# ChenFengTsai/dreamerv3-torch

Hardware: AMD Instinct MI355X
Metric: imagination-steps/sec (higher is better)
Workload: dtype f32; 1 GPU; cfg2: dmc_vision 64x64x3 synthetic replay, RSSM deter=512 hidden=512 stoch=32x32, continuous actor (6), imag_gradient dynamics, batch 16 x seq 64 per GPU, horizon 15; one step = full Dreamer._train update (world model + actor + critic fwd/bwd, gradient all-reduce, 3x clip+Adam); global_batch=16, seq_len=64, horizon=15, parallelism=dp1

## Files before the change

### dreamerv3-torch_amd/csrc/conv.hip

```cpp
#include <stdlib.h>

#include "mfma_gemm.h"
#include "l16_tile.h"
#include "dv3_common.h"

namespace dv3 {

struct FastDiv {
  int d, shift;
  __host__ __device__ static FastDiv make(int d) {
    FastDiv f{d, -1};
    if (d > 0 && (d & (d - 1)) == 0) {
      int s = 0;
      while ((1 << s) < d) ++s;
      f.shift = s;
    }
    return f;
  }
  __device__ __forceinline__ long quot(long x) const { return shift >= 0 ? (x >> shift) : x / d; }
  __device__ __forceinline__ int rem(long x) const { return shift >= 0 ? (int)(x & (d - 1)) : (int)(x % d); }
  __device__ __forceinline__ int quot(int x) const { return shift >= 0 ? (x >> shift) : x / d; }
  __device__ __forceinline__ int rem(int x) const { return shift >= 0 ? (x & (d - 1)) : x % d; }
};

// ... 509 lines not shown
  f32x4n acc[2][RN];
#pragma unroll
  for (int t = 0; t < 2; ++t)
#pragma unroll
    for (int c = 0; c < RN; ++c) acc[t][c] = (f32x4n){0.f, 0.f, 0.f, 0.f};
  const int chunks = (K + 15) >> 4;
  f32x4n a0[2], b0[RN], a1[2], b1[RN];
  float m0[2], m1[2];
  auto load = [&](f32x4n (&a)[2], f32x4n (&b)[RN], float (&msk)[2], int c) {
    if (c >= chunks) return;
    const int k = (c << 4) + 4 * q;
    const int tap = dC.quot(k), ci = dC.rem(k);
    const int ky = tap >> 2, kx = tap & 3;
#pragma unroll
    for (int t = 0; t < 2; ++t) {
      const int iy = y0[t] + ky, ix = x0[t] + kx;
      const bool ok = base[t] >= 0 && iy >= 0 && iy < p.H && ix >= 0 && ix < p.W;
      const float* src = ok ? p.x + base[t] + ((long)iy * p.W + ix) * p.Ci + ci : p.x;
      a[t] = *reinterpret_cast<const f32x4u*>(src);
      msk[t] = ok ? 1.f : 0.f;
    }
#pragma unroll
    for (int cc = 0; cc < RN; ++cc) b[cc] = *reinterpret_cast<const f32x4u*>(wrow[cc] + k);
  };
  auto compute = [&](const f32x4n (&a)[2], const f32x4n (&b)[RN], const float (&msk)[2], int c) {
    if (c >= chunks) return;
#pragma unroll
    for (int g = 0; g < 4; ++g)
#pragma unroll
      for (int t = 0; t < 2; ++t) {
        const float av = a[t][g] * msk[t];
#pragma unroll
        for (int cc = 0; cc < RN; ++cc)
          acc[t][cc] = __builtin_amdgcn_mfma_f32_16x16x4f32(av, b[cc][g] * bmask[cc], acc[t][cc], 0, 0, 0);
      }
  };
  load(a0, b0, m0, 0);
  for (int c = 0; c < chunks; c += 2) {
    load(a1, b1, m1, c + 1);
    compute(a0, b0, m0, c);
    load(a0, b0, m0, c + 2);
    compute(a1, b1, m1, c + 1);
  }
#pragma unroll
  for (int t = 0; t < 2; ++t)
#pragma unroll
    for (int r = 0; r < 4; ++r) {
      const long m = row0 + 16 * t + 4 * q + r;
      if (m >= M) continue;
      float* orow = p.y + m * p.Co;
#pragma unroll
      for (int cc = 0; cc < RN; ++cc) {
        const int co = 16 * cc + i;
        if (co < p.Co) orow[co] = p.accumulate ? (orow[co] + acc[t][cc][r]) : acc[t][cc][r];
      }
    }
}

struct WgradParams {
  const float* dy;
  const float* x;
  float* dw;
  int Nimg, H, W, Ci, Co;
  int tiles_m, tiles_n, splits, chunk;
  int xcd_group;
};

template <class TS, bool C3 = false>
__global__ __launch_bounds__(kThreads) void conv_wgrad_kernel(WgradParams p) {
  __shared__ __attribute__((aligned(16))) float lds[TS::lds_floats];
  using ATile = DenseTile<TS::BM, TS::BK, false>;
  using BTile = WgradBTile<TS::BN, TS::BK, C3>;
  const int OH = p.H / 2, OW = p.W / 2;
  const long rows = (long)p.Nimg * OH * OW;
  DenseOperand<false> aop{p.dy, nullptr, (long)p.Co, 0, p.Co, (int)rows, (int)rows, true};
  WgradB bop{p.x, p.H, p.W, p.Ci, OH, OW, rows, 16 * p.Ci, FastDiv::make(OW), FastDiv::make(OH),
             FastDiv::make(p.Ci), FastDiv::make(4 * p.Ci)};
  const int tiles = p.tiles_m * p.tiles_n;
  int tile, split;
  if (p.xcd_group) {
    const int xcd = blockIdx.x & 7, j = blockIdx.x >> 3;
    split = (j / tiles) * 8 + xcd;
    tile = j % tiles;
    if (split >= p.splits) return;
  } else {
    tile = blockIdx.x % tiles;
    split = blockIdx.x / tiles;
  }
  const int m0 = (tile / p.tiles_n) * TS::BM, n0 = (tile % p.tiles_n) * TS::BN;
  const long kb = (long)split * p.chunk;
  long ke = kb + p.chunk;
  if (ke > rows) ke = rows;
  f32x16 acc[TS::TM][TS::TN];
  bool owner;
  mfma_mainloop<TS, ATile, BTile>(aop, bop, m0, n0, (int)kb, (int)ke, lds, acc, owner);
  if (kb >= ke || !owner) return;
  const int tid = threadIdx.x, wave = (tid >> 6) % (TS::WM * TS::WN), lane = tid & 63;
  const int wm = wave / TS::WN, wn = wave % TS::WN, col_l = lane & 31, h = lane >> 5;
#pragma unroll
  for (int a = 0; a < TS::TM; ++a)
#pragma unroll
    for (int b = 0; b < TS::TN; ++b) {
      const int j = n0 + (wn * TS::TN + b) * 32 + col_l;
      if (j >= 16 * p.Ci) continue;
#pragma unroll
      for (int r = 0; r < 16; ++r) {
        const int co = m0 + (wm * TS::TM + a) * 32 + (r & 3) + 8 * (r >> 2) + 4 * h;
        if (co < p.Co) atomicAdd(p.dw + (long)co * (16 * p.Ci) + j, acc[a][b][r]);
      }
    }
}

__global__ void unpack_conv_wgrad_kernel(float* __restrict__ packed, float* __restrict__ dw, int Co, int Ci) {
  const long total = (long)Co * Ci * 16;
  for (long i = (long)blockIdx.x * blockDim.x + threadIdx.x; i < total; i += (long)gridDim.x * blockDim.x) {
    const int ci = (int)(i % Ci);
    long t = i / Ci;
    const int kx = (int)(t % 4);
    t /= 4;
    const int ky = (int)(t % 4);
    const long co = t / 4;
    dw[((co * Ci + ci) * 4 + ky) * 4 + kx] += packed[i];
    packed[i] = 0.f;
  }
}

__global__ void pack_conv_w_kernel(const float* __restrict__ w, float* __restrict__ wp, int Co, int Ci) {
  const long total = (long)Co * Ci * 16;
  for (long i = (long)blockIdx.x * blockDim.x + threadIdx.x; i < total; i += (long)gridDim.x * blockDim.x) {
    const int ci = (int)(i % Ci);
    long t = i / Ci;
    const int kx = (int)(t % 4);
    t /= 4;
    const int ky = (int)(t % 4);
    const long co = t / 4;
    wp[i] = w[((co * Ci + ci) * 4 + ky) * 4 + kx];
  }
}
__global__ void pack_convT_w_kernel(const float* __restrict__ w, float* __restrict__ wp, int Ci, int Co) {
  const long total = 4L * Co * 4 * Ci;
  for (long i = (long)blockIdx.x * blockDim.x + threadIdx.x; i < total; i += (long)gridDim.x * blockDim.x) {
    const int ci = (int)(i % Ci);
    long t = i / Ci;
    const int b = (int)(t % 2);
    t /= 2;
    const int a = (int)(t % 2);
    t /= 2;
    const int co = (int)(t % Co);
    const int cls = (int)(t / Co);
    const int py = cls >> 1, px = cls & 1;
    const int ky = 1 - py + 2 * a, kx = 1 - px + 2 * b;
    wp[i] = w[(((long)ci * Co + co) * 4 + ky) * 4 + kx];
  }
}


typedef float f4a __attribute__((ext_vector_type(4), aligned(4)));

template <int CW>
__global__ __launch_bounds__(256) void conv_s2_c3_kernel(const float* __restrict__ x, const float* __restrict__ w,
                                                         float* __restrict__ y, int Nimg, int H, int W,
                                                         int accumulate) {
  const int OH = H / 2, OW = W / 2;
  const long total = (long)Nimg * OH * OW;
  for (long p = (long)blockIdx.x * blockDim.x + threadIdx.x; p < total; p += (long)gridDim.x * blockDim.x) {
    const int ox = (int)(p % OW);
    const long t = p / OW;
    const int oy = (int)(t % OH);
    const long n = t / OH;
    float in[4][12];
#pragma unroll
    for (int ky = 0; ky < 4; ++ky) {
      const int iy = 2 * oy - 1 + ky;
      const bool rowok = iy >= 0 && iy < H;
      const float* row = x + ((n * H + (rowok ? iy : 0)) * W) * 3;
#pragma unroll
      for (int kx = 0; kx < 4; ++kx) {
        const int ix = 2 * ox - 1 + kx;
        const bool ok = rowok && ix >= 0 && ix < W;
        const float* q = row + (ok ? ix : 0) * 3;
        const float m = ok ? 1.f : 0.f;
        in[ky][kx * 3 + 0] = q[0] * m;
        in[ky][kx * 3 + 1] = q[1] * m;
        in[ky][kx * 3 + 2] = q[2] * m;
      }
    }
    float* out = y + p * CW;
#pragma unroll 1
    for (int c0 = 0; c0 < CW; c0 += 4) {
      f4a acc = {0.f, 0.f, 0.f, 0.f};
#pragma unroll
      for (int e = 0; e < 4; ++e) {
        const float* wc = w + (long)(c0 + e) * 48;
        float a = 0.f;
#pragma unroll
        for (int c = 0; c < 3; ++c)
#pragma unroll
          for (int ky = 0; ky < 4; ++ky)
#pragma unroll
            for (int kx = 0; kx < 4; ++kx) a += in[ky][kx * 3 + c] * wc[(c * 4 + ky) * 4 + kx];
        acc[e] = a;
      }
      f4a* o = reinterpret_cast<f4a*>(out + c0);
      if (accumulate) acc += *o;
      *o = acc;
    }
  }
}

template <int CW>
__global__ __launch_bounds__(256) void conv_s2_c3_mfma_kernel(const float* __restrict__ x, const float* __restrict__ w,
                                                              float* __restrict__ y, int Nimg, int H, int W,
                                                              int accumulate) {
  constexpr int LD = 52, TN = CW / 16;
  __shared__ __attribute__((aligned(16))) float As[128 * LD];
  __shared__ __attribute__((aligned(16))) float Bs[CW * LD];
  const int tid = threadIdx.x, wave = tid >> 6, lane = tid & 63;
  const int i = lane & 15, q = lane >> 4;
  const int OH = H / 2, OW = W / 2;
  const long total = (long)Nimg * OH * OW;
  const long p0 = (long)blockIdx.x * 128;
  for (int e = tid; e < CW * 48; e += 256) {
    const int co = e / 48, r = e - co * 48;
    const int c = r >> 4, ky = (r >> 2) & 3, kx = r & 3;
    Bs[co * LD + ky * 12 + kx * 3 + c] = w[e];
  }
  {
    const int pl = tid >> 1, kyb = (tid & 1) * 2;
    const long p = p0 + pl;
    const bool pv = p < total;
    const long pc = pv ? p : 0;
    const int ox = (int)(pc % OW);
    const long t = pc / OW;
    const int oy = (int)(t % OH);
    const long n = t / OH;
    const bool edge = (ox == 0) || (ox == OW - 1);
#pragma unroll
    for (int kk = 0; kk < 2; ++kk) {
      const int ky = kyb + kk;
      const int iy = 2 * oy - 1 + ky;
      const bool rowok = pv && iy >= 0 && iy < H;
      float* dst = &As[pl * LD + ky * 12];
      f32x4 v0 = {0.f, 0.f, 0.f, 0.f}, v1 = v0, v2 = v0;
      if (rowok) {
        const float* row = x + ((n * H + iy) * W) * 3;
        if (!edge) {
          const float* src = row + (2 * ox - 1) * 3;
          v0 = *reinterpret_cast<const f32x4u*>(src);
          v1 = *reinterpret_cast<const f32x4u*>(src + 4);
          v2 = *reinterpret_cast<const f32x4u*>(src + 8);
        } else {
          float tmp[12];
#pragma unroll
          for (int j = 0; j < 12; ++j) {
            const int ix = 2 * ox - 1 + j / 3;
            tmp[j] = (ix >= 0 && ix < W) ? row[ix * 3 + j % 3] : 0.f;
          }
          v0 = (f32x4){tmp[0], tmp[1], tmp[2], tmp[3]};
          v1 = (f32x4){tmp[4], tmp[5], tmp[6], tmp[7]};
          v2 = (f32x4){tmp[8], tmp[9], tmp[10], tmp[11]};
        }
      }
      *reinterpret_cast<f32x4*>(dst) = v0;
      *reinterpret_cast<f32x4*>(dst + 4) = v1;
      *reinterpret_cast<f32x4*>(dst + 8) = v2;
    }
  }
  __syncthreads();
  f32x4 acc[2][TN];
#pragma unroll
  for (int a = 0; a < 2; ++a)
#pragma unroll
    for (int b = 0; b < TN; ++b) acc[a][b] = (f32x4){0.f, 0.f, 0.f, 0.f};
#pragma unroll
  for (int c = 0; c < 3; ++c) {
    f32x4 af[2], bf[TN];
#pragma unroll
    for (int a = 0; a < 2; ++a) af[a] = *reinterpret_cast<const f32x4*>(&As[(wave * 32 + 16 * a + i) * LD + 16 * c + 4 * q]);
#pragma unroll
    for (int b = 0; b < TN; ++b) bf[b] = *reinterpret_cast<const f32x4*>(&Bs[(16 * b + i) * LD + 16 * c + 4 * q]);
#pragma unroll
    for (int g = 0; g < 4; ++g)
#pragma unroll
      for (int a = 0; a < 2; ++a)
#pragma unroll
        for (int b = 0; b < TN; ++b)
          acc[a][b] = __builtin_amdgcn_mfma_f32_16x16x4f32(af[a][g], bf[b][g], acc[a][b], 0, 0, 0);
  }
#pragma unroll
  for (int a = 0; a < 2; ++a)
#pragma unroll
    for (int b = 0; b < TN; ++b)
#pragma unroll
      for (int r = 0; r < 4; ++r) {
        const long p = p0 + wave * 32 + 16 * a + 4 * q + r;
        if (p < total) {
          float* o = y + p * CW + 16 * b + i;
          const float v = acc[a][b][r];
          *o = accumulate ? (*o + v) : v;
        }
      }
}

template <int CW>
__global__ __launch_bounds__(256) void convT_s2_c3_kernel(const float* __restrict__ x, const float* __restrict__ w,
                                                          const float* __restrict__ bias, float out_add,
                                                          float* __restrict__ y, int Nimg, int IH, int IW,
                                                          int accumulate) {
  const long total = (long)Nimg * IH * IW;
  const int OW = 2 * IW, OH = 2 * IH;
  for (long p = (long)blockIdx.x * blockDim.x + threadIdx.x; p < total; p += (long)gridDim.x * blockDim.x) {
    const int x2 = (int)(p % IW);
    const long t = p / IW;
    const int y2 = (int)(t % IH);
    const long n = t / IH;
    float acc[2][2][3];
#pragma unroll
    for (int py = 0; py < 2; ++py)
#pragma unroll
      for (int px = 0; px < 2; ++px)
#pragma unroll
        for (int co = 0; co < 3; ++co) acc[py][px][co] = 0.f;
#pragma unroll 1
    for (int c0 = 0; c0 < CW; c0 += 4) {
      f4a in[3][3];
#pragma unroll
      for (int dy = 0; dy < 3; ++dy)
#pragma unroll
        for (int dx = 0; dx < 3; ++dx) {
          const int iy = y2 + dy - 1, ix = x2 + dx - 1;
          const bool ok = iy >= 0 && iy < IH && ix >= 0 && ix < IW;
          const float* q = x + (((n * IH + (ok ? iy : 0)) * IW + (ok ? ix : 0)) * CW) + c0;
          in[dy][dx] = *reinterpret_cast<const f4a*>(q) * (ok ? 1.f : 0.f);
        }
#pragma unroll
      for (int e = 0; e < 4; ++e) {
        const float* wc = w + (long)(c0 + e) * 48;
#pragma unroll
        for (int py = 0; py < 2; ++py)
#pragma unroll
          for (int a = 0; a < 2; ++a)
#pragma unroll
            for (int px = 0; px < 2; ++px)
#pragma unroll
              for (int b = 0; b < 2; ++b) {
                const float v = in[py - a + 1][px - b + 1][e];
                const int ky = 1 - py + 2 * a, kx = 1 - px + 2 * b;
#pragma unroll
                for (int co = 0; co < 3; ++co) acc[py][px][co] += v * wc[(co * 4 + ky) * 4 + kx];
              }
      }
    }
    const float b0 = (bias ? bias[0] : 0.f) + out_add, b1 = (bias ? bias[1] : 0.f) + out_add,
                b2 = (bias ? bias[2] : 0.f) + out_add;
#pragma unroll
    for (int py = 0; py < 2; ++py) {
      float* o = y + (((n * OH + 2 * y2 + py) * OW) + 2 * x2) * 3;
      float v[6] = {acc[py][0][0] + b0, acc[py][0][1] + b1, acc[py][0][2] + b2,
                    acc[py][1][0] + b0, acc[py][1][1] + b1, acc[py][1][2] + b2};
#pragma unroll
      for (int e = 0; e < 6; ++e) o[e] = accumulate ? (o[e] + v[e]) : v[e];
    }
  }
}

template <int CW>
__global__ __launch_bounds__(256) void convT_s2_c3_mfma_kernel(const float* __restrict__ x, const float* __restrict__ w,
                                                               const float* __restrict__ bias, float out_add,
                                                               float* __restrict__ y, int Nimg, int IH, int IW,
                                                               int accumulate) {
  constexpr int NCH = CW / 16;
  constexpr int RB = (18 * 18 + 15) / 16;
  constexpr int LDP = 52;
  __shared__ float P[RB * 16 * LDP];
  const int tid = threadIdx.x, wave = tid >> 6, lane = tid & 63;
  const int i = lane & 15, q = lane >> 4;
  const int tx_n = IW / 16, ty_n = IH / 16;
  const int img = blockIdx.x / (tx_n * ty_n), trem = blockIdx.x % (tx_n * ty_n);
  const int ty = trem / tx_n, tx = trem % tx_n;
  const float* xin = x + (long)img * IH * IW * CW;
  f32x4 bf[NCH][3];
#pragma unroll
  for (int c = 0; c < NCH; ++c)
#pragma unroll
    for (int b = 0; b < 3; ++b)
#pragma unroll
      for (int g = 0; g < 4; ++g) bf[c][b][g] = w[(long)(16 * c + 4 * q + g) * 48 + 16 * b + i];
  constexpr int RPW = (RB + 3) / 4;
  constexpr int JB = NCH <= 2 ? RPW : 2;
  for (int j0 = 0; j0 < RPW; j0 += JB) {
    f32x4 af[JB][NCH];
    float msk[JB];
#pragma unroll
    for (int j = 0; j < JB; ++j) {
      const int pl = (wave + 4 * (j0 + j)) * 16 + i;
      const int ly = pl / 18, lx = pl % 18;
      const int gy = ty * 16 + ly - 1, gx = tx * 16 + lx - 1;
      const bool ok = pl < 18 * 18 && gy >= 0 && gy < IH && gx >= 0 && gx < IW;
      const float* src = xin + ((long)(ok ? gy : 0) * IW + (ok ? gx : 0)) * CW + 4 * q;
#pragma unroll
      for (int c = 0; c < NCH; ++c) af[j][c] = *reinterpret_cast<const f32x4u*>(src + 16 * c);
      msk[j] = ok ? 1.f : 0.f;
    }
#pragma unroll
    for (int j = 0; j < JB; ++j) {
      const int rbk = wave + 4 * (j0 + j);
      if (rbk >= RB) continue;
      f32x4 acc[3];
#pragma unroll
      for (int b = 0; b < 3; ++b) acc[b] = (f32x4){0.f, 0.f, 0.f, 0.f};
#pragma unroll
      for (int c = 0; c < NCH; ++c)
#pragma unroll
        for (int g = 0; g < 4; ++g)
#pragma unroll
          for (int b = 0; b < 3; ++b)
            acc[b] = __builtin_amdgcn_mfma_f32_16x16x4f32(af[j][c][g] * msk[j], bf[c][b][g], acc[b], 0, 0, 0);
#pragma unroll
      for (int r = 0; r < 4; ++r)
#pragma unroll
        for (int b = 0; b < 3; ++b) P[(rbk * 16 + 4 * q + r) * LDP + 16 * b + i] = acc[b][r];
    }
  }
  __syncthreads();
  const int OH = 2 * IH, OW = 2 * IW;
  const float bb[3] = {(bias ? bias[0] : 0.f) + out_add, (bias ? bias[1] : 0.f) + out_add, (bias ? bias[2] : 0.f) + out_add};
#pragma unroll 4
  for (int f = tid; f < 32 * 32 * 3; f += 256) {
    const int oy = f / 96, col = f % 96;
    const int ox = col / 3, c = col % 3;
    const int ky0 = (oy + 1) & 1, kx0 = (ox + 1) & 1;
    float v = bb[c];
#pragma unroll
    for (int dy = 0; dy < 2; ++dy)
#pragma unroll
      for (int dx = 0; dx < 2; ++dx) {
        const int ky = ky0 + 2 * dy, kx = kx0 + 2 * dx;
        const int ly = (oy + 3 - ky) >> 1, lx = (ox + 3 - kx) >> 1;
        v += P[(ly * 18 + lx) * LDP + c * 16 + ky * 4 + kx];
      }
    float* o = y + (((long)img * OH + 32 * ty + oy) * OW + 32 * tx) * 3 + col;
    *o = accumulate ? (*o + v) : v;
  }
}

template <int CW>
__global__ __launch_bounds__(256) void conv_wgrad_c3_kernel(const float* __restrict__ coarse,
                                                            const float* __restrict__ fine, float* __restrict__ dw,
                                                            int Nimg, int H, int W) {
  constexpr int MA = CW / 16, LDC = CW + 16;
  constexpr int CV = 256 * (CW / 4) / 256;
  constexpr int FN = 34 * 34 * 3, FV = (FN + 255) / 256;
  extern __shared__ __attribute__((aligned(16))) float wlds[];
  float* cs = wlds;
  float* fs = wlds + 256 * LDC;
  const int tid = threadIdx.x, wave = tid >> 6, lane = tid & 63;
  const int i = lane & 15, q = lane >> 4;
  const int OH = H / 2, OW = W / 2;
  const int tx_n = OW / 16, ty_n = OH / 16;
  const int tiles = Nimg * tx_n * ty_n;
  f32x4 cv[CV];
  float fv[FV];
  auto gload = [&](int tile) {
    const int img = tile / (tx_n * ty_n), trem = tile % (tx_n * ty_n);
    const int ty = trem / tx_n, tx = trem % tx_n;
    const float* cbase = coarse + (((long)img * OH + ty * 16) * OW + tx * 16) * CW;
#pragma unroll
    for (int j = 0; j < CV; ++j) {
      const int f = tid + 256 * j;
      const int pix = f / (CW / 4), c4 = (f % (CW / 4)) * 4;
      cv[j] = *reinterpret_cast<const f32x4u*>(cbase + ((long)(pix >> 4) * OW + (pix & 15)) * CW + c4);
    }
    const float* fbase = fine + (long)img * H * W * 3;
#pragma unroll
    for (int j = 0; j < FV; ++j) {
      const int f = tid + 256 * j;
      const int fy = f / 102, fr = f % 102;
      const int gy = 32 * ty - 1 + fy, gxc = (32 * tx - 1) * 3 + fr;
      const bool ok = f < FN && gy >= 0 && gy < H && gxc >= 0 && gxc < 3 * W;
      fv[j] = ok ? fbase[(long)gy * W * 3 + gxc] : 0.f;
    }
  };
  auto lstore = [&]() {
#pragma unroll
    for (int j = 0; j < CV; ++j) {
      const int f = tid + 256 * j;
      *reinterpret_cast<f32x4*>(&cs[(f / (CW / 4)) * LDC + (f % (CW / 4)) * 4]) = cv[j];
    }
#pragma unroll
    for (int j = 0; j < FV; ++j) {
      const int f = tid + 256 * j;
      if (f < FN) fs[f] = fv[j];
    }
  };
  f32x4 acc[MA][3];
#pragma unroll
  for (int a = 0; a < MA; ++a)
#pragma unroll
    for (int b = 0; b < 3; ++b) acc[a][b] = (f32x4){0.f, 0.f, 0.f, 0.f};
  int boff[3];
#pragma unroll
  for (int b = 0; b < 3; ++b) {
    const int n = 16 * b + i;
    boff[b] = (((n >> 2) & 3) * 34 + (n & 3)) * 3 + (n >> 4);
  }
  int tile = blockIdx.x;
  if (tile < tiles) gload(tile);
  for (; tile < tiles; tile += gridDim.x) {
    __syncthreads();
    lstore();
    __syncthreads();
    if (tile + (int)gridDim.x < tiles) gload(tile + gridDim.x);
#pragma unroll 4
    for (int s = 0; s < 16; ++s) {
      const int pk = wave * 64 + 4 * s + q;
      const int cy = pk >> 4, cx = pk & 15;
      float av[MA], bv[3];
#pragma unroll
      for (int a = 0; a < MA; ++a) av[a] = cs[pk * LDC + 16 * a + i];
      const int fo = (2 * cy * 34 + 2 * cx) * 3;
#pragma unroll
      for (int b = 0; b < 3; ++b) bv[b] = fs[fo + boff[b]];
#pragma unroll
      for (int a = 0; a < MA; ++a)
#pragma unroll
        for (int b = 0; b < 3; ++b) acc[a][b] = __builtin_amdgcn_mfma_f32_16x16x4f32(av[a], bv[b], acc[a][b], 0, 0, 0);
    }
  }
  __syncthreads();
  float* red = cs;
#pragma unroll
  for (int a = 0; a < MA; ++a)
#pragma unroll
    for (int b = 0; b < 3; ++b)
#pragma unroll
      for (int r = 0; r < 4; ++r) red[(wave * MA * 3 + a * 3 + b) * 256 + r * 64 + lane] = acc[a][b][r];
  __syncthreads();
  for (int e = tid; e < MA * 3 * 256; e += 256) {
    const int blk = e >> 8, x = e & 255;
    const int a = blk / 3, b = blk % 3;
    const int r = x >> 6, l = x & 63;
    const int cc = 16 * a + 4 * (l >> 4) + r, n = 16 * b + (l & 15);
    const float v = red[e] + red[MA * 3 * 256 + e] + red[2 * MA * 3 * 256 + e] + red[3 * MA * 3 * 256 + e];
    atomicAdd(dw + (long)cc * 48 + n, v);
  }
}

template <int CF, int CC>
__global__ __launch_bounds__(512) void conv_wgrad_tile_kernel(const float* __restrict__ coarse,
                                                              const float* __restrict__ fine, float* __restrict__ partial,
                                                              int Nimg, int H, int W) {
  constexpr int NT = 512, MA = CC / 16, NH = CF / 16, LDC = CC + 16, LDF = CF + 8;
  constexpr int CVN = 64 * (CC / 4), CV = (CVN + NT - 1) / NT;
  constexpr int FVN = 18 * 18 * (CF / 4), FV = (FVN + NT - 1) / NT;
  extern __shared__ __attribute__((aligned(16))) float wlds[];
  float* cs = wlds;
  float* fs = wlds + 64 * LDC;
  const int tid = threadIdx.x, wave = tid >> 6, lane = tid & 63;
  const int i = lane & 15, q = lane >> 4;
  const int OH = H / 2, OW = W / 2;
  const int tx_n = OW / 8, ty_n = OH / 8;
  const int tiles = Nimg * tx_n * ty_n;
  f32x4 cv[CV], fv[FV];
  auto gload = [&](int tile) {
    const int img = tile / (tx_n * ty_n), trem = tile % (tx_n * ty_n);
    const int ty = trem / tx_n, tx = trem % tx_n;
    const float* cbase = coarse + (((long)img * OH + ty * 8) * OW + tx * 8) * CC;
#pragma unroll
    for (int j = 0; j < CV; ++j) {
      const int f = tid + NT * j;
      const int pix = (f < CVN ? f : 0) / (CC / 4), c4 = (f % (CC / 4)) * 4;
      cv[j] = *reinterpret_cast<const f32x4u*>(cbase + ((long)(pix >> 3) * OW + (pix & 7)) * CC + c4);
    }
    const float* fbase = fine + (long)img * H * W * CF;
#pragma unroll
    for (int j = 0; j < FV; ++j) {
      const int f = tid + NT * j;
      const int pix = f / (CF / 4), c4 = (f % (CF / 4)) * 4;
      const int fy = pix / 18, fx = pix % 18;
      const int gy = 16 * ty - 1 + fy, gx = 16 * tx - 1 + fx;
      const bool ok = f < FVN && gy >= 0 && gy < H && gx >= 0 && gx < W;
      fv[j] = *reinterpret_cast<const f32x4u*>(fbase + ((long)(ok ? gy : 0) * W + (ok ? gx : 0)) * CF + c4);
      if (!ok) fv[j] = (f32x4){0.f, 0.f, 0.f, 0.f};
    }
  };
  auto lstore = [&]() {
#pragma unroll
    for (int j = 0; j < CV; ++j) {
      const int f = tid + NT * j;
      if (f < CVN) *reinterpret_cast<f32x4*>(&cs[(f / (CC / 4)) * LDC + (f % (CC / 4)) * 4]) = cv[j];
    }
#pragma unroll
    for (int j = 0; j < FV; ++j) {
      const int f = tid + NT * j;
      if (f < FVN) *reinterpret_cast<f32x4*>(&fs[(f / (CF / 4)) * LDF + (f % (CF / 4)) * 4]) = fv[j];
    }
  };
  f32x4 acc[MA][2 * NH];
#pragma unroll
  for (int a = 0; a < MA; ++a)
#pragma unroll
    for (int b = 0; b < 2 * NH; ++b) acc[a][b] = (f32x4){0.f, 0.f, 0.f, 0.f};
  int boff[2 * NH];
#pragma unroll
  for (int b = 0; b < 2 * NH; ++b) {
    const int tap = 2 * wave + b / NH;
    boff[b] = ((tap >> 2) * 18 + (tap & 3)) * LDF + 16 * (b % NH) + i;
  }
  int tile = blockIdx.x;
  if (tile < tiles) gload(tile);
  for (; tile < tiles; tile += gridDim.x) {
    __syncthreads();
    lstore();
    __syncthreads();
    if (tile + (int)gridDim.x < tiles) gload(tile + gridDim.x);
#pragma unroll 4
    for (int s = 0; s < 16; ++s) {
      const int pk = 4 * s + q;
      const int cy = pk >> 3, cx = pk & 7;
      float av[MA], bv[2 * NH];
#pragma unroll
      for (int a = 0; a < MA; ++a) av[a] = cs[pk * LDC + 16 * a + i];
      const int fo = (2 * cy * 18 + 2 * cx) * LDF;
#pragma unroll
      for (int b = 0; b < 2 * NH; ++b) bv[b] = fs[fo + boff[b]];
#pragma unroll
      for (int a = 0; a < MA; ++a)
#pragma unroll
        for (int b = 0; b < 2 * NH; ++b) acc[a][b] = __builtin_amdgcn_mfma_f32_16x16x4f32(av[a], bv[b], acc[a][b], 0, 0, 0);
    }
  }
  float* out = partial + (long)blockIdx.x * CC * 16 * CF;
#pragma unroll
  for (int a = 0; a < MA; ++a)
#pragma unroll
    for (int b = 0; b < 2 * NH; ++b) {
      const int tap = 2 * wave + b / NH, cf = 16 * (b % NH) + i;
#pragma unroll
      for (int r = 0; r < 4; ++r) out[(long)(16 * a + 4 * q + r) * (16 * CF) + tap * CF + cf] = acc[a][b][r];
    }
}

__global__ __launch_bounds__(256) void conv_wgrad_tile_reduce_kernel(const float* __restrict__ partial, float* __restrict__ dw,
                                                                     int G, int CC, int CF) {
  const int total = CC * 16 * CF;
  const int e = blockIdx.x * 256 + threadIdx.x;
  if (e >= total) return;
  float s0 = 0.f, s1 = 0.f, s2 = 0.f, s3 = 0.f;
  int g = 0;
  for (; g + 3 < G; g += 4) {
    s0 += partial[(long)g * total + e];
    s1 += partial[(long)(g + 1) * total + e];
    s2 += partial[(long)(g + 2) * total + e];
    s3 += partial[(long)(g + 3) * total + e];
  }
  for (; g < G; ++g) s0 += partial[(long)g * total + e];
  const int cf = e % CF, tap = (e / CF) % 16, cc = e / (16 * CF);
  dw[(((long)cc * CF + cf) * 4 + (tap >> 2)) * 4 + (tap & 3)] += (s0 + s1) + (s2 + s3);
}

using C128 = TileShape<2, 2, 2, 2, 16>;
using C128K32 = TileShape<2, 2, 2, 2, 32>;
using C64 = TileShape<2, 2, 1, 1, 32>;
using C128x32 = TileShape<4, 1, 1, 1, 32>;
using C32x64S = TileShape<1, 2, 1, 1, 64, 2>;

}

using namespace dv3;

static bool pow2_spatial(int H, int W) { return H > 0 && W > 0 && (H % 2) == 0 && (W % 2) == 0; }

extern "C" int dv3_pack_conv_weight(const float* w, float* wp, int Co, int Ci, int transposed, void* stream) {
  if (!w || !wp || Co <= 0 || Ci <= 0) return DV3_ERR_ARG;
  const long total = 16L * Co * Ci;
  unsigned blocks = (unsigned)((total + 255) / 256);
  if (blocks > 2048) blocks = 2048;
  if (transposed) hipLaunchKernelGGL(pack_convT_w_kernel, dim3(blocks), dim3(256), 0, (hipStream_t)stream, w, wp, Ci, Co);
  else hipLaunchKernelGGL(pack_conv_w_kernel, dim3(blocks), dim3(256), 0, (hipStream_t)stream, w, wp, Co, Ci);
  return (int)hipGetLastError();
}

template <int BM, int BN, bool TR, int VAR = 3>
__global__ __launch_bounds__(256) void conv_s2_l16_kernel(ConvParams p) {
  constexpr int TM = BM / 32, TN = BN / 32;
  __shared__ __attribute__((aligned(16))) float As[2][BM * L16_LD];
  __shared__ __attribute__((aligned(16))) float Bs[2][BN * L16_LD];
  const int tid = threadIdx.x, wave = tid >> 6, lane = tid & 63;
  const int i = lane & 15, q = lane >> 4;
  const int wm = wave >> 1, wn = wave & 1;
  int cls = 0, lin = blockIdx.x;
  if constexpr (TR) {
    if (!convT_tile_class(p.tiles_m * p.tiles_n, lin, cls)) return;
  }
  const int py = cls >> 1, px = cls & 1;
  const int RH = TR ? p.H : (p.H >> 1), RW = TR ? p.W : (p.W >> 1);
  const long M = (long)p.Nimg * RH * RW;
  const int K = (TR ? 4 : 16) * p.Ci;
  if constexpr (!TR) {
    const int tiles = p.tiles_m * p.tiles_n;
    if ((p.tiles_m & 7) == 0) lin = (blockIdx.x & 7) * (tiles >> 3) + (blockIdx.x >> 3);
  }
  const int tm = lin / p.tiles_n, tn = lin % p.tiles_n;
  const long m0 = (long)tm * BM;
  const int n0 = tn * BN;
  constexpr int NA = l16_slots<BM>, NB = l16_slots<BN>;
  const int c4 = l16_stage_k(tid);
  const float* abase[NA];
  int iy0[NA], ix0[NA];
  bool rowok[NA];
#pragma unroll
  for (int j = 0; j < NA; ++j) {
    const long m = m0 + l16_stage_row(tid, j);
    rowok[j] = m < M;
    const long mm = rowok[j] ? m : 0;
    const int rx = (int)(mm % RW);
    const long t = mm / RW;
    const int ry = (int)(t % RH);
    const long n = t / RH;
    iy0[j] = TR ? ry + py : 2 * ry - 1;
    ix0[j] = TR ? rx + px : 2 * rx - 1;
    abase[j] = p.x + n * p.H * p.W * p.Ci + c4;
  }
  const float* bsrc[NB];
#pragma unroll
  for (int j = 0; j < NB; ++j) {
    const int col = n0 + l16_stage_row(tid, j);
    bsrc[j] = p.wp + (long)cls * p.Co * K + (long)(col < p.Co ? col : 0) * K + c4;
  }
  f32x4 ra[NA], rb[NB];
  bool aok[NA];
  auto load = [&](int, int k0) {
    const int tap = k0 / p.Ci, ci0 = k0 - tap * p.Ci;
    const int ty = TR ? -(tap >> 1) : (tap >> 2), tx = TR ? -(tap & 1) : (tap & 3);
#pragma unroll
    for (int j = 0; j < NA; ++j) {
      const int iy = iy0[j] + ty, ix = ix0[j] + tx;
      aok[j] = rowok[j] && iy >= 0 && iy < p.H && ix >= 0 && ix < p.W;
      const float* src = aok[j] ? abase[j] + ((long)iy * p.W + ix) * p.Ci + ci0 : p.x;
      ra[j] = *reinterpret_cast<const f32x4*>(src);
    }
#pragma unroll
    for (int j = 0; j < NB; ++j) rb[j] = *reinterpret_cast<const f32x4*>(bsrc[j] + k0);
  };
// ... 129 lines not shown
      const int f = tid + NT * j;
      const int pix = f / (CI / 4), c4 = (f % (CI / 4)) * 4;
      const int ly = pix / 18, lx = pix % 18;
      const int gy = ty * 16 + ly - 1, gx = tx * 16 + lx - 1;
      const bool ok = f < XV && gy >= 0 && gy < p.H && gx >= 0 && gx < p.W;
      xv[j] = *reinterpret_cast<const f32x4u*>(xin + ((long)(ok ? gy : 0) * p.W + (ok ? gx : 0)) * CI + c4);
      if (!ok) xv[j] = (f32x4){0.f, 0.f, 0.f, 0.f};
    }
#pragma unroll
    for (int j = 0; j < XJ; ++j) {
      const int f = tid + NT * j;
      if (f < XV) *reinterpret_cast<f32x4*>(&xs[(f / (CI / 4)) * LDX + (f % (CI / 4)) * 4]) = xv[j];
    }
  }
  wstore();
  __syncthreads();
  const int OH = 2 * p.H, OW = 2 * p.W;
  const float bias0 = (p.bias && i < p.Co) ? p.bias[i] : 0.f;
  const float bias1 = (p.bias && 16 + i < p.Co) ? p.bias[16 + i] : 0.f;
  for (int cls = 0; cls < 4; ++cls) {
    const int py = cls >> 1, px = cls & 1;
    if (cls < 3) wload(cls + 1);
    f32x4 acc[RPW][2];
#pragma unroll
    for (int a = 0; a < RPW; ++a)
#pragma unroll
      for (int b = 0; b < 2; ++b) acc[a][b] = (f32x4){0.f, 0.f, 0.f, 0.f};
#pragma unroll
    for (int tap = 0; tap < 4; ++tap) {
      const int ta = tap >> 1, tb = tap & 1;
      const int xoff = ((RPW * wave + py - ta + 1) * 18 + (i + px - tb + 1)) * LDX + 4 * q;
      const int woff = i * LDW + tap * CI + 4 * q;
#pragma unroll
      for (int c = 0; c < NCH; ++c) {
        f32x4 af[RPW], bf[2];
#pragma unroll
        for (int a = 0; a < RPW; ++a) af[a] = *reinterpret_cast<const f32x4*>(&xs[xoff + a * 18 * LDX + 16 * c]);
#pragma unroll
        for (int b = 0; b < 2; ++b) bf[b] = *reinterpret_cast<const f32x4*>(&ws[woff + 16 * b * LDW + 16 * c]);
#pragma unroll
        for (int g = 0; g < 4; ++g)
#pragma unroll
          for (int a = 0; a < RPW; ++a)
#pragma unroll
            for (int b = 0; b < 2; ++b)
              acc[a][b] = __builtin_amdgcn_mfma_f32_16x16x4f32(af[a][g], bf[b][g], acc[a][b], 0, 0, 0);
      }
    }
#pragma unroll
    for (int a = 0; a < RPW; ++a) {
      const int oy = 2 * (ty * 16 + RPW * wave + a) + py;
#pragma unroll
      for (int r = 0; r < 4; ++r) {
        const int ox = 2 * (tx * 16 + 4 * q + r) + px;
        float* orow = p.y + (((long)img * OH + oy) * OW + ox) * p.Co;
#pragma unroll
        for (int b = 0; b < 2; ++b) {
          const int co = 16 * b + i;
          if (co < p.Co) {
            const float val = acc[a][b][r] + (b ? bias1 : bias0) + p.out_add;
            orow[co] = p.accumulate ? (orow[co] + val) : val;
          }
        }
      }
    }
    if (cls < 3) {
      __syncthreads();
      wstore();
      __syncthreads();
    }
  }
}


__global__ void im2col_s2_kernel(const float* __restrict__ x, float* __restrict__ cols, int Nimg, int H, int W, int C) {
  const int OH = H >> 1, OW = W >> 1;
  const long K = 16L * C, total = (long)Nimg * OH * OW * K;
  for (long e = (long)blockIdx.x * blockDim.x + threadIdx.x; e < total; e += (long)gridDim.x * blockDim.x) {
    const int k = (int)(e % K);
    long m = e / K;
    const int kx = k & 3, ky = (k >> 2) & 3, ci = k >> 4;
    const int ox = (int)(m % OW);
    m /= OW;
    const int oy = (int)(m % OH);
    const long n = m / OH;
    const int iy = 2 * oy - 1 + ky, ix = 2 * ox - 1 + kx;
    const bool ok = iy >= 0 && iy < H && ix >= 0 && ix < W;
    cols[e] = ok ? x[((n * H + iy) * W + ix) * C + ci] : 0.f;
  }
}

extern "C" int dv3_im2col_s2(const float* x, float* cols, int Nimg, int H, int W, int C, void* stream) {
  if (Nimg <= 0) return 0;
  if (!x || !cols || C <= 0 || H <= 0 || W <= 0 || (H & 1) || (W & 1)) return DV3_ERR_ARG;
  const long total = (long)Nimg * (H / 2) * (W / 2) * 16 * C;
  unsigned blocks = (unsigned)((total + 255) / 256);
  if (blocks > 4096) blocks = 4096;
  hipLaunchKernelGGL(im2col_s2_kernel, dim3(blocks), dim3(256), 0, (hipStream_t)stream, x, cols, Nimg, H, W, C);
  return (int)hipGetLastError();
}

#define DV3_CONV_L16_LAUNCH(BM_, BN_, TR_)                                                                       \
  l16_with_var<3>([&](auto var) {                                                                                \
    hipLaunchKernelGGL((conv_s2_l16_kernel<BM_, BN_, TR_, decltype(var)::value>), grid, dim3(256), 0, s, p);    \
  })

extern "C" int dv3_conv_s2_fwd(const float* x, const float* w_packed, float* y, int Nimg, int H, int W, int Ci, int Co,
                               int accumulate, void* stream) {
  if (Nimg <= 0) return 0;
  if (!x || !w_packed || !y || Ci <= 0 || Co <= 0 || !pow2_spatial(H, W)) return DV3_ERR_ARG;
  ConvParams p{x, w_packed, y, nullptr, 0.f, Nimg, H, W, Ci, Co, 0, 0, accumulate};
  const long M = (long)Nimg * (H / 2) * (W / 2);
  if (M > 0x7fffffffL - 256) return DV3_ERR_ARG;
  hipStream_t s = (hipStream_t)stream;
  auto go = [&](auto ts) {
    using TS = decltype(ts);
    p.tiles_m = (int)((M + TS::BM - 1) / TS::BM);
    p.tiles_n = (Co + TS::BN - 1) / TS::BN;
    hipLaunchKernelGGL((conv_s2_kernel<TS>), dim3(p.tiles_m * p.tiles_n), dim3(kThreads), 0, s, p);
  };
  const long tiles128 = ((M + 127) / 128) * ((Co + 127) / 128);
  static const int env_l16 = DV3_ENV_INT("DV3_CONV_L16", 1);
  if (env_l16 && (Ci % 32) == 0 && Co >= 64 && ((uintptr_t)x % 16) == 0 && ((uintptr_t)w_packed % 16) == 0) {
    const int bn = (env_l16 != 3 && (Co % 128) == 0) ? 128 : (env_l16 != 3 && (Co % 96) == 0) ? 96 : 64;
    const bool big = bn != 64 && (env_l16 == 4 || (env_l16 == 1 && ((M + 127) / 128) * (Co / bn) >= 448));
    const int bm = big ? 128 : 64;
    p.tiles_m = (int)((M + bm - 1) / bm);
    p.tiles_n = (Co + bn - 1) / bn;
    const dim3 grid((unsigned)(p.tiles_m * p.tiles_n));
    if (bn == 128 && big) DV3_CONV_L16_LAUNCH(128, 128, false);
    else if (bn == 128) DV3_CONV_L16_LAUNCH(64, 128, false);
    else if (bn == 96 && big) DV3_CONV_L16_LAUNCH(128, 96, false);
    else if (bn == 96) DV3_CONV_L16_LAUNCH(64, 96, false);
    else DV3_CONV_L16_LAUNCH(64, 64, false);
    return (int)hipGetLastError();
  }
  static const int env_direct = DV3_ENV_INT("DV3_CONV_DIRECT", 64);
  if ((Ci & 3) == 0 && Co <= env_direct && Co <= 128) {
    const dim3 grid((unsigned)((M + 127) / 128));
    if (Co <= 32) hipLaunchKernelGGL(conv_s2_direct_kernel<2>, grid, dim3(256), 0, s, p);
    else if (Co <= 64) hipLaunchKernelGGL(conv_s2_direct_kernel<4>, grid, dim3(256), 0, s, p);
    else hipLaunchKernelGGL(conv_s2_direct_kernel<8>, grid, dim3(256), 0, s, p);
    return (int)hipGetLastError();
  }
  if (Co <= 32) go(C128x32{});
  else if (Co <= 64 || tiles128 <= 256) go(C64{});
  else go(C128{});
  return (int)hipGetLastError();
}

extern "C" int dv3_convT_s2_fwd(const float* x, const float* w_packed, const float* bias, float out_add, float* y,
                                int Nimg, int IH, int IW, int Ci, int Co, int accumulate, void* stream) {
  if (Nimg <= 0) return 0;
  if (!x || !w_packed || !y || Ci <= 0 || Co <= 0 || IH <= 0 || IW <= 0) return DV3_ERR_ARG;
  ConvParams p{x, w_packed, y, bias, out_add, Nimg, IH, IW, Ci, Co, 0, 0, accumulate};
  const long M = (long)Nimg * IH * IW;
  if (M > 0x7fffffffL - 256) return DV3_ERR_ARG;
  hipStream_t s = (hipStream_t)stream;
  auto go = [&](auto ts) {
    using TS = decltype(ts);
    p.tiles_m = (int)((M + TS::BM - 1) / TS::BM);
    p.tiles_n = (Co + TS::BN - 1) / TS::BN;
    hipLaunchKernelGGL((convT_s2_kernel<TS>), dim3(p.tiles_m * p.tiles_n, 4), dim3(kThreads), 0, s, p);
  };
  static const int env_tile = DV3_ENV_INT("DV3_CONVT_TILE", 1);
  if (env_tile && Co <= 32 && (Ci == 16 || Ci == 32 || Ci == 48 || Ci == 64) && (IH % 16) == 0 && (IW % 16) == 0) {
    const dim3 grid((unsigned)((long)Nimg * (IH / 16) * (IW / 16)));
    const size_t lds = (size_t)(18 * 18 * (Ci + 8) + 32 * (4 * Ci + 8)) * sizeof(float);
#define DV3_CT(CI_)                                                                                              \
  {                                                                                                              \
    static unsigned long long seen[4] = {0, 0, 0, 0};                                                            \
    if (dv3_first_on_device(seen))                                                                               \
      (void)hipFuncSetAttribute((const void*)convT_s2_tile_kernel<CI_>, hipFuncAttributeMaxDynamicSharedMemorySize, (int)lds); \
    hipLaunchKernelGGL((convT_s2_tile_kernel<CI_>), grid, dim3(512), lds, s, p);                                  \
  }
    if (Ci == 16) DV3_CT(16) else if (Ci == 32) DV3_CT(32) else if (Ci == 48) DV3_CT(48) else DV3_CT(64)
#undef DV3_CT
    return (int)hipGetLastError();
  }
  static const int env_l16 = DV3_ENV_INT("DV3_CONVT_L16", 1);
  const bool co96 = (Co % 96) == 0 && (Co % 128) != 0 && env_l16 != 3;
  if (env_l16 && (Ci % 32) == 0 && (Co >= (env_l16 == 2 ? 32 : 128) || (co96 && env_l16 != 5)) &&
      ((uintptr_t)x % 16) == 0 && ((uintptr_t)w_packed % 16) == 0) {
    const int bn = (Co % 128) == 0 && env_l16 != 3 ? 128 : co96 ? 96 : (Co % 64) == 0 ? 64 : 32;
    const bool big = (bn == 128 || bn == 96) && ((M + 127) / 128) * (Co / bn) * 4 >= 448;
    const int bm = (bn == 32 || big) ? 128 : 64;
    p.tiles_m = (int)((M + bm - 1) / bm);
    p.tiles_n = (Co + bn - 1) / bn;
    const dim3 grid(convT_grid((long)p.tiles_m * p.tiles_n));
    if (bn == 128 && big) DV3_CONV_L16_LAUNCH(128, 128, true);
    else if (bn == 128) DV3_CONV_L16_LAUNCH(64, 128, true);
    else if (bn == 96 && big) DV3_CONV_L16_LAUNCH(128, 96, true);
    else if (bn == 96) DV3_CONV_L16_LAUNCH(64, 96, true);
    else if (bn == 64) DV3_CONV_L16_LAUNCH(64, 64, true);
    else DV3_CONV_L16_LAUNCH(128, 32, true);
    return (int)hipGetLastError();
  }
  static const int env_direct = DV3_ENV_INT("DV3_CONVT_DIRECT", 128);
  if ((Ci & 3) == 0 && Co <= env_direct && Co <= 128) {
    const dim3 grid(convT_grid((M + 127) / 128));
    if (Co <= 32) hipLaunchKernelGGL(convT_s2_direct_kernel<2>, grid, dim3(256), 0, s, p);
    else if (Co <= 64) hipLaunchKernelGGL(convT_s2_direct_kernel<4>, grid, dim3(256), 0, s, p);
    else hipLaunchKernelGGL(convT_s2_direct_kernel<8>, grid, dim3(256), 0, s, p);
    return (int)hipGetLastError();
  }
  if (Co <= 32) go(C128x32{});
  else if (Co <= 64) go(C64{});
  else go(C128{});
  return (int)hipGetLastError();
}

extern "C" int dv3_conv_s2_wgrad(const float* coarse, const float* fine, float* dw_packed, float* dw, int Nimg, int H,
                                 int W, int Cfine, int Ccoarse, void* stream) {
  if (Nimg <= 0) return 0;
  if (!coarse || !fine || !dw || !dw_packed || Cfine <= 0 || Ccoarse <= 0 || !pow2_spatial(H, W)) return DV3_ERR_ARG;
  const long rows = (long)Nimg * (H / 2) * (W / 2);
  if (rows > 0x7fffffffL - 4096) return DV3_ERR_ARG;
  static const int env_c3w = DV3_ENV_INT("DV3_C3W_TILE", 1);
  if (env_c3w && Cfine == 3 && (Ccoarse == 32 || Ccoarse == 96) && ((H / 2) % 16) == 0 && ((W / 2) % 16) == 0) {
    const long tiles = (long)Nimg * (H / 32) * (W / 32);
    const size_t lds = (size_t)(256 * (Ccoarse + 16) + 34 * 34 * 3) * sizeof(float);
    const unsigned grid = (unsigned)(tiles < 512 ? tiles : 512);
    if (Ccoarse == 32) {
      hipLaunchKernelGGL((conv_wgrad_c3_kernel<32>), dim3(grid), dim3(256), lds, (hipStream_t)stream, coarse, fine, dw, Nimg, H, W);
    } else {
      static unsigned long long seen[4] = {0, 0, 0, 0};
      if (dv3_first_on_device(seen))
        (void)hipFuncSetAttribute((const void*)conv_wgrad_c3_kernel<96>, hipFuncAttributeMaxDynamicSharedMemorySize, (int)lds);
      hipLaunchKernelGGL((conv_wgrad_c3_kernel<96>), dim3(grid), dim3(256), lds, (hipStream_t)stream, coarse, fine, dw, Nimg, H, W);
    }
    return (int)hipGetLastError();
  }
  WgradParams p{coarse, fine, dw_packed, Nimg, H, W, Cfine, Ccoarse, 0, 0, 0, 0, 0};
  static const int env_group = DV3_ENV_INT("DV3_WGRAD_XCD", 1);
  auto go = [&](auto ts, long target_wgs) {
    using TS = decltype(ts);
    p.tiles_m = (Ccoarse + TS::BM - 1) / TS::BM;
    p.tiles_n = (16 * Cfine + TS::BN - 1) / TS::BN;
    const int tiles = p.tiles_m * p.tiles_n;
    long splits = (target_wgs + tiles - 1) / tiles;
    const long max_splits = (rows + 511) / 512;
    if (splits > max_splits) splits = max_splits;
    if (splits < 1) splits = 1;
    long chunk = (rows + splits - 1) / splits;
    chunk = ((chunk + TS::BK - 1) / TS::BK) * TS::BK;
    splits = (rows + chunk - 1) / chunk;
    p.splits = (int)splits;
    p.chunk = (int)chunk;
    p.xcd_group = (env_group && splits >= 8) ? 1 : 0;
    const long gsplits = p.xcd_group ? (splits + 7) / 8 * 8 : splits;
    if (Cfine == 3) hipLaunchKernelGGL((conv_wgrad_kernel<TS, true>), dim3((unsigned)(tiles * gsplits)), dim3(kThreads), 0, (hipStream_t)stream, p);
    else hipLaunchKernelGGL((conv_wgrad_kernel<TS, false>), dim3((unsigned)(tiles * gsplits)), dim3(kThreads), 0, (hipStream_t)stream, p);
  };
  static const int env_k32 = DV3_ENV_INT("DV3_WGRAD_K32", 1);
  static const int env_wgs = DV3_ENV_INT("DV3_WGRAD_WGS", 0);
  auto target128 = [&](int bm, int bn) {
    if (env_wgs > 0) return (long)env_wgs;
    const long tiles = (long)((Ccoarse + bm - 1) / bm) * ((16 * Cfine + bn - 1) / bn);
    const long by_rows = tiles * ((rows + 3071) / 3072);
    return by_rows > 512 ? by_rows : 512L;
  };
  if (Ccoarse >= 128 && env_k32) go(C128K32{}, target128(128, 128));
  else if (Ccoarse >= 128) go(C128{}, target128(128, 128));
  else if (Ccoarse <= 32) go(C32x64S{}, 1024);
  else go(C64{}, 1024);
  const long total = 16L * Ccoarse * Cfine;
  unsigned ub = (unsigned)((total + 255) / 256);
  if (ub > 1024) ub = 1024;
  hipLaunchKernelGGL(unpack_conv_wgrad_kernel, dim3(ub), dim3(256), 0, (hipStream_t)stream, dw_packed, dw, Ccoarse, Cfine);
  return (int)hipGetLastError();
}

extern "C" int dv3_conv_s2_wgrad_tile_scratch(int Nimg, int H, int W, int Cfine, int Ccoarse) {
  if (Cfine != 32 || Ccoarse != 64 || H <= 0 || W <= 0 || (H % 16) != 0 || (W % 16) != 0 || Nimg <= 0) return 0;
  const long tiles = (long)Nimg * (H / 16) * (W / 16);
  return (int)((tiles < 256 ? tiles : 256) * (long)Ccoarse * 16 * Cfine);
}
extern "C" int dv3_conv_s2_wgrad_tile(const float* coarse, const float* fine, float* partial, float* dw, int Nimg, int H,
                                      int W, int Cfine, int Ccoarse, void* stream) {
  if (Nimg <= 0) return 0;
  if (!coarse || !fine || !partial || !dw || dv3_conv_s2_wgrad_tile_scratch(Nimg, H, W, Cfine, Ccoarse) == 0)
    return DV3_ERR_ARG;
  const long tiles = (long)Nimg * (H / 16) * (W / 16);
  const int G = (int)(tiles < 256 ? tiles : 256);
  const size_t lds = (size_t)(64 * (64 + 16) + 18 * 18 * (32 + 8)) * sizeof(float);
  static unsigned long long seen[4] = {0, 0, 0, 0};
  if (dv3_first_on_device(seen))
    (void)hipFuncSetAttribute((const void*)conv_wgrad_tile_kernel<32, 64>, hipFuncAttributeMaxDynamicSharedMemorySize, (int)lds);
  hipStream_t s = (hipStream_t)stream;
  hipLaunchKernelGGL((conv_wgrad_tile_kernel<32, 64>), dim3(G), dim3(512), lds, s, coarse, fine, partial, Nimg, H, W);
  hipLaunchKernelGGL(conv_wgrad_tile_reduce_kernel, dim3((64 * 16 * 32 + 255) / 256), dim3(256), 0, s, partial, dw, G, 64, 32);
  return (int)hipGetLastError();
}

extern "C" int dv3_conv_s2_c3_fwd(const float* x, const float* w, float* y, int Nimg, int H, int W, int CW,
                                  int accumulate, void* stream) {
  if (Nimg <= 0) return 0;
  if (!x || !w || !y || !pow2_spatial(H, W)) return DV3_ERR_ARG;
  const long total = (long)Nimg * (H / 2) * (W / 2);
  unsigned blocks = (unsigned)((total + 255) / 256);
  if (blocks > 16384) blocks = 16384;
  hipStream_t s = (hipStream_t)stream;
  static const int env_mfma = DV3_ENV_INT("DV3_C3_MFMA", 1);
  if (env_mfma && (CW == 32 || CW == 96) && total < 0x7fffffffL * 64) {
    const dim3 grid((unsigned)((total + 127) / 128));
    if (CW == 32) hipLaunchKernelGGL((conv_s2_c3_mfma_kernel<32>), grid, dim3(256), 0, s, x, w, y, Nimg, H, W, accumulate);
    else hipLaunchKernelGGL((conv_s2_c3_mfma_kernel<96>), grid, dim3(256), 0, s, x, w, y, Nimg, H, W, accumulate);
    return (int)hipGetLastError();
  }
  if (CW == 32) hipLaunchKernelGGL((conv_s2_c3_kernel<32>), dim3(blocks), dim3(256), 0, s, x, w, y, Nimg, H, W, accumulate);
  else if (CW == 96) hipLaunchKernelGGL((conv_s2_c3_kernel<96>), dim3(blocks), dim3(256), 0, s, x, w, y, Nimg, H, W, accumulate);
  else return DV3_ERR_ARG;
  return (int)hipGetLastError();
}
extern "C" int dv3_convT_s2_c3_fwd(const float* x, const float* w, const float* bias, float out_add, float* y,
                                   int Nimg, int IH, int IW, int CW, int accumulate, void* stream) {
  if (Nimg <= 0) return 0;
  if (!x || !w || !y || IH <= 0 || IW <= 0) return DV3_ERR_ARG;
  const long total = (long)Nimg * IH * IW;
  unsigned blocks = (unsigned)((total + 255) / 256);
  if (blocks > 16384) blocks = 16384;
  hipStream_t s = (hipStream_t)stream;
  static const int env_c3t = DV3_ENV_INT("DV3_C3T_MFMA", 1);
  if (env_c3t && (IH % 16) == 0 && (IW % 16) == 0 && (CW == 32 || CW == 96)) {
    const dim3 grid((unsigned)((long)Nimg * (IH / 16) * (IW / 16)));
    if (CW == 32) hipLaunchKernelGGL((convT_s2_c3_mfma_kernel<32>), grid, dim3(256), 0, s, x, w, bias, out_add, y, Nimg, IH, IW, accumulate);
    else hipLaunchKernelGGL((convT_s2_c3_mfma_kernel<96>), grid, dim3(256), 0, s, x, w, bias, out_add, y, Nimg, IH, IW, accumulate);
    return (int)hipGetLastError();
  }
  if (CW == 32) hipLaunchKernelGGL((convT_s2_c3_kernel<32>), dim3(blocks), dim3(256), 0, s, x, w, bias, out_add, y, Nimg, IH, IW, accumulate);
  else if (CW == 96) hipLaunchKernelGGL((convT_s2_c3_kernel<96>), dim3(blocks), dim3(256), 0, s, x, w, bias, out_add, y, Nimg, IH, IW, accumulate);
  else return DV3_ERR_ARG;
  return (int)hipGetLastError();
}
```

Baseline: 1.216 million imagination-steps/s.

## Add LDS-banded MFMA kernel for 3-channel stride-2 conv and halve convT tile height

Adds a new forward kernel for the first stride-2 conv on 3-channel input. It stages a band of input rows in LDS, with two shifted copies so loads stay 16-byte aligned, and keeps weights in LDS. Each block then computes 128 output pixels with MFMA and writes results as vector stores. The matching transposed-conv MFMA kernel now uses 8-row tiles instead of 16, which doubles the grid and shrinks LDS use per block. It also swaps the MFMA operand order so accumulators can be stored to LDS as f32x4. The cost is more halo rows recomputed per output for the transposed conv, and an extra specialised code path that only covers some widths.

```diff
diff --git a/dreamerv3-torch_amd/csrc/conv.hip b/dreamerv3-torch_amd/csrc/conv.hip
--- a/dreamerv3-torch_amd/csrc/conv.hip
+++ b/dreamerv3-torch_amd/csrc/conv.hip
@@ -835,6 +835,101 @@
       }
 }
 
+constexpr int kC3BandMax = 6 * (3 * 128 + 8);
+
+template <int CW>
+__global__ __launch_bounds__(256) void conv_s2_c3_band_kernel(const float* __restrict__ x, const float* __restrict__ w,
+                                                              float* __restrict__ y, int H, int W, int lgOW,
+                                                              int accumulate) {
+  constexpr int LD = 52, TN = CW / 16;
+  __shared__ __attribute__((aligned(16))) float Xs[2 * kC3BandMax];
+  __shared__ __attribute__((aligned(16))) float Bs[CW * LD];
+  const int tid = threadIdx.x, wave = tid >> 6, lane = tid & 63;
+  const int i = lane & 15, q = lane >> 4;
+  const int OW = 1 << lgOW, R = 128 >> lgOW, NR = 2 * R + 2, RS = 3 * W + 8;
+  const int tpi = (H / 2) / R;
+  const int n = blockIdx.x / tpi, oy0 = (blockIdx.x - n * tpi) * R;
+  const float* xin = x + (long)n * H * W * 3;
+  constexpr int NJ = 3;
+  const int V = 3 << (lgOW - 1);
+  f32x4 xv[NJ];
+#pragma unroll
+  for (int j = 0; j < NJ; ++j) {
+    const int f = tid + 256 * j;
+    const int rr = (f >> (lgOW - 1)) / 3, m = f - rr * V;
+    const int iy = 2 * oy0 - 1 + rr;
+    xv[j] = (f32x4){0.f, 0.f, 0.f, 0.f};
+    if (rr < NR && iy >= 0 && iy < H) xv[j] = *reinterpret_cast<const f32x4*>(xin + ((long)iy * W * 3 + 4 * m));
+  }
+  for (int e = tid; e < CW * 48; e += 256) {
+    const int co = e / 48, r = e - co * 48;
+    const int c = r >> 4, ky = (r >> 2) & 3, kx = r & 3;
+    Bs[co * LD + ky * 12 + kx * 3 + c] = w[e];
+  }
+  if (tid < NR) {
+    float* r0 = &Xs[tid * RS];
+    float* r1 = r0 + kC3BandMax;
+#pragma unroll
+    for (int e = 0; e < 3; ++e) {
+      r0[e] = 0.f;
+      r0[3 * W + 3 + e] = 0.f;
+      r1[2 + e] = 0.f;
+      r1[3 * W + 5 + e] = 0.f;
+    }
+  }
+#pragma unroll
+  for (int j = 0; j < NJ; ++j) {
+    const int f = tid + 256 * j;
+    const int rr = (f >> (lgOW - 1)) / 3, m = f - rr * V;
+    if (rr < NR) {
+      float* d0 = &Xs[rr * RS + 3 + 4 * m];
+      float* d1 = d0 + kC3BandMax + 2;
+#pragma unroll
+      for (int e = 0; e < 4; ++e) {
+        d0[e] = xv[j][e];
+        d1[e] = xv[j][e];
+      }
+    }
+  }
+  __syncthreads();
+  int xo[2];
+#pragma unroll
+  for (int a = 0; a < 2; ++a) {
+    const int pl = wave * 32 + 16 * a + i;
+    const int r = pl >> lgOW, ox = pl & (OW - 1);
+    xo[a] = 2 * r * RS + 6 * ox + ((ox & 1) ? kC3BandMax + 2 : 0);
+  }
+  f32x4 acc[2][TN];
+#pragma unroll
+  for (int a = 0; a < 2; ++a)
+#pragma unroll
+    for (int b = 0; b < TN; ++b) acc[a][b] = (f32x4){0.f, 0.f, 0.f, 0.f};
+#pragma unroll
+  for (int c = 0; c < 3; ++c) {
+    const int k0 = 16 * c + 4 * q, ky = k0 / 12, rem = k0 - 12 * ky;
+    f32x4 xf[2], wf[TN];
+#pragma unroll
+    for (int a = 0; a < 2; ++a) xf[a] = *reinterpret_cast<const f32x4*>(&Xs[xo[a] + ky * RS + rem]);
+#pragma unroll
+    for (int b = 0; b < TN; ++b) wf[b] = *reinterpret_cast<const f32x4*>(&Bs[(16 * b + i) * LD + 16 * c + 4 * q]);
+#pragma unroll
+    for (int g = 0; g < 4; ++g)
+#pragma unroll
+      for (int a = 0; a < 2; ++a)
+#pragma unroll
+        for (int b = 0; b < TN; ++b)
+          acc[a][b] = __builtin_amdgcn_mfma_f32_16x16x4f32(wf[b][g], xf[a][g], acc[a][b], 0, 0, 0);
+  }
+  float* yt = y + ((long)blockIdx.x * 128 + wave * 32 + i) * CW + 4 * q;
+#pragma unroll
+  for (int a = 0; a < 2; ++a)
+#pragma unroll
+    for (int b = 0; b < TN; ++b) {
+      f32x4* o = reinterpret_cast<f32x4*>(yt + (long)16 * a * CW + 16 * b);
+      *o = accumulate ? (*o + acc[a][b]) : acc[a][b];
+    }
+}
+
 template <int CW>
 __global__ __launch_bounds__(256) void convT_s2_c3_kernel(const float* __restrict__ x, const float* __restrict__ w,
                                                           const float* __restrict__ bias, float out_add,
@@ -903,12 +998,13 @@
                                                                float* __restrict__ y, int Nimg, int IH, int IW,
                                                                int accumulate) {
   constexpr int NCH = CW / 16;
-  constexpr int RB = (18 * 18 + 15) / 16;
+  constexpr int TR = 8, NPIX = (TR + 2) * 18;
+  constexpr int RB = (NPIX + 15) / 16;
   constexpr int LDP = 52;
-  __shared__ float P[RB * 16 * LDP];
+  __shared__ __attribute__((aligned(16))) float P[RB * 16 * LDP];
   const int tid = threadIdx.x, wave = tid >> 6, lane = tid & 63;
   const int i = lane & 15, q = lane >> 4;
-  const int tx_n = IW / 16, ty_n = IH / 16;
+  const int tx_n = IW / 16, ty_n = IH / TR;
   const int img = blockIdx.x / (tx_n * ty_n), trem = blockIdx.x % (tx_n * ty_n);
   const int ty = trem / tx_n, tx = trem % tx_n;
   const float* xin = x + (long)img * IH * IW * CW;
@@ -928,8 +1024,8 @@
     for (int j = 0; j < JB; ++j) {
       const int pl = (wave + 4 * (j0 + j)) * 16 + i;
       const int ly = pl / 18, lx = pl % 18;
-      const int gy = ty * 16 + ly - 1, gx = tx * 16 + lx - 1;
-      const bool ok = pl < 18 * 18 && gy >= 0 && gy < IH && gx >= 0 && gx < IW;
+      const int gy = ty * TR + ly - 1, gx = tx * 16 + lx - 1;
+      const bool ok = pl < NPIX && gy >= 0 && gy < IH && gx >= 0 && gx < IW;
       const float* src = xin + ((long)(ok ? gy : 0) * IW + (ok ? gx : 0)) * CW + 4 * q;
 #pragma unroll
       for (int c = 0; c < NCH; ++c) af[j][c] = *reinterpret_cast<const f32x4u*>(src + 16 * c);
@@ -948,18 +1044,16 @@
         for (int g = 0; g < 4; ++g)
 #pragma unroll
           for (int b = 0; b < 3; ++b)
-            acc[b] = __builtin_amdgcn_mfma_f32_16x16x4f32(af[j][c][g] * msk[j], bf[c][b][g], acc[b], 0, 0, 0);
-#pragma unroll
-      for (int r = 0; r < 4; ++r)
-#pragma unroll
-        for (int b = 0; b < 3; ++b) P[(rbk * 16 + 4 * q + r) * LDP + 16 * b + i] = acc[b][r];
+            acc[b] = __builtin_amdgcn_mfma_f32_16x16x4f32(bf[c][b][g], af[j][c][g] * msk[j], acc[b], 0, 0, 0);
+#pragma unroll
+      for (int b = 0; b < 3; ++b) *reinterpret_cast<f32x4*>(&P[(rbk * 16 + i) * LDP + 16 * b + 4 * q]) = acc[b];
     }
   }
   __syncthreads();
   const int OH = 2 * IH, OW = 2 * IW;
   const float bb[3] = {(bias ? bias[0] : 0.f) + out_add, (bias ? bias[1] : 0.f) + out_add, (bias ? bias[2] : 0.f) + out_add};
 #pragma unroll 4
-  for (int f = tid; f < 32 * 32 * 3; f += 256) {
+  for (int f = tid; f < 2 * TR * 32 * 3; f += 256) {
     const int oy = f / 96, col = f % 96;
     const int ox = col / 3, c = col % 3;
     const int ky0 = (oy + 1) & 1, kx0 = (ox + 1) & 1;
@@ -972,7 +1066,7 @@
         const int ly = (oy + 3 - ky) >> 1, lx = (ox + 3 - kx) >> 1;
         v += P[(ly * 18 + lx) * LDP + c * 16 + ky * 4 + kx];
       }
-    float* o = y + (((long)img * OH + 32 * ty + oy) * OW + 32 * tx) * 3 + col;
+    float* o = y + (((long)img * OH + 2 * TR * ty + oy) * OW + 32 * tx) * 3 + col;
     *o = accumulate ? (*o + v) : v;
   }
 }
@@ -1708,6 +1802,16 @@
   if (blocks > 16384) blocks = 16384;
   hipStream_t s = (hipStream_t)stream;
   static const int env_mfma = DV3_ENV_INT("DV3_C3_MFMA", 1);
+  static const int env_band = DV3_ENV_INT("DV3_C3_BAND", 1);
+  const int OW = W / 2;
+  if (env_mfma && env_band && (CW == 32 || CW == 96) && total < 0x7fffffffL * 64 && (OW == 16 || OW == 32 || OW == 64) &&
+      (H / 2) % (128 / OW) == 0 && (((uintptr_t)x | (uintptr_t)y) & 15) == 0) {
+    const dim3 grid((unsigned)(total / 128));
+    const int lgOW = OW == 16 ? 4 : OW == 32 ? 5 : 6;
+    if (CW == 32) hipLaunchKernelGGL((conv_s2_c3_band_kernel<32>), grid, dim3(256), 0, s, x, w, y, H, W, lgOW, accumulate);
+    else hipLaunchKernelGGL((conv_s2_c3_band_kernel<96>), grid, dim3(256), 0, s, x, w, y, H, W, lgOW, accumulate);
+    return (int)hipGetLastError();
+  }
   if (env_mfma && (CW == 32 || CW == 96) && total < 0x7fffffffL * 64) {
     const dim3 grid((unsigned)((total + 127) / 128));
     if (CW == 32) hipLaunchKernelGGL((conv_s2_c3_mfma_kernel<32>), grid, dim3(256), 0, s, x, w, y, Nimg, H, W, accumulate);
@@ -1729,7 +1833,7 @@
   hipStream_t s = (hipStream_t)stream;
   static const int env_c3t = DV3_ENV_INT("DV3_C3T_MFMA", 1);
   if (env_c3t && (IH % 16) == 0 && (IW % 16) == 0 && (CW == 32 || CW == 96)) {
-    const dim3 grid((unsigned)((long)Nimg * (IH / 16) * (IW / 16)));
+    const dim3 grid((unsigned)((long)Nimg * (IH / 8) * (IW / 16)));
     if (CW == 32) hipLaunchKernelGGL((convT_s2_c3_mfma_kernel<32>), grid, dim3(256), 0, s, x, w, bias, out_add, y, Nimg, IH, IW, accumulate);
     else hipLaunchKernelGGL((convT_s2_c3_mfma_kernel<96>), grid, dim3(256), 0, s, x, w, bias, out_add, y, Nimg, IH, IW, accumulate);
     return (int)hipGetLastError();
```

Result: faster. 1.231 million imagination-steps/s, median of 6 (+1.2%).
